# EugenHotaj/pytorch-generative

Measured on AMD Instinct MI355X. Metric: training images/sec (ImageGPT 8-block/4-head/16-embed, 28x28x1), higher is better.
Workload: dtype f32; 1 GPU; BASELINE.json configs[1]: ImageGPT 8 blocks / 4 heads / 16 embed on 28x28x1 binarised-MNIST-shaped synthetic; one step = zero_grad + fwd + BCE + bwd + global grad-norm + Adam + lr decay (reference trainer.py:173-193); per_gpu_batch=1024, global_batch=1024, parallelism=dp1, launch=hipGraph replay

## Files before the change

include/pg_hip.h:

```cpp
#ifndef PG_HIP_H_
#define PG_HIP_H_

#include <stddef.h>
#include <stdint.h>

#ifdef __cplusplus
extern "C" {
#endif

#define PG_ABI_VERSION 1

#define PG_EINVAL (-1)
#define PG_ESHAPE (-2)

#define PG_MAX_TAPS 64

#define PG_ACT_NONE 0
#define PG_ACT_RELU 1
#define PG_ACT_ELU 2
#define PG_ACT_GELU 3
#define PG_ACT_ELU_OUT 4

#define PG_GATE_TANH 0
#define PG_GATE_IDENTITY 1
// ... 70 lines not shown
                       long k_bs, long v_bs, long o_bs, long do_bs, long dq_bs, long dk_bs,
                       long dv_bs, int strict, void* stream);

int pg_causal_attn_bwd_dq(const float* q, const float* k, const float* v, const float* o,
                          const float* d_o, const float* lse2, float* delta, float* dq, float* dk,
                          float* dv, int N, int heads, int L, int dk_dim, int dv_dim, long q_bs,
                          long k_bs, long v_bs, long o_bs, long do_bs, long dq_bs, long dk_bs,
                          long dv_bs, int strict, void* stream);
int pg_causal_attn_bwd_dkv(const float* q, const float* k, const float* v, const float* o,
                           const float* d_o, const float* lse2, float* delta, float* dq, float* dk,
                           float* dv, int N, int heads, int L, int dk_dim, int dv_dim, long q_bs,
                           long k_bs, long v_bs, long o_bs, long do_bs, long dq_bs, long dk_bs,
                           long dv_bs, int strict, void* stream);

int pg_attn_fused_bwd(int enable);

#define PG_FEATURE_IDENTITY 0
#define PG_FEATURE_ELU1 1
size_t pg_linear_attn_workspace_floats(int N, int heads, int L, int dk, int dv, int backward);
int pg_linear_attn_fwd(const float* q, const float* k, const float* v, float* out, float* den, float* ws,
                       size_t ws_floats, int N, int heads, int L, int dk, int dv, long q_bs, long kv_bs,
                       long o_bs, int feature, void* stream);
int pg_linear_attn_bwd(const float* q, const float* k, const float* v, const float* out, const float* den,
                       const float* g, float* dq, float* dk, float* dv, float* ws, size_t ws_floats, int N,
                       int heads, int L, int dk_dim, int dv_dim, long q_bs, long kv_bs, long o_bs, int feature,
                       void* stream);

size_t pg_masked_linear_workspace_floats(int N, int in, int out, int dgrad);
int pg_masked_linear_fwd(const float* x, float* w, const float* b, const int* deg_in, const int* deg_out, int strict,
                         float* y, int N, int in, int out, int relu, float* ws, size_t ws_floats, void* stream);
// ... 145 lines not shown
```

pytorch-generative_amd/csrc/attention.hip:

```cpp
#include <stdlib.h>

#include "attention_args.h"

namespace {

constexpr float NEG_BIG = -1.0e30f;
constexpr float POS_BIG = 1.0e30f;
constexpr int QPL = 2;

using AttnArgs = PgAttnArgs;

__device__ __forceinline__ float fast_exp2(float x) { return __builtin_amdgcn_exp2f(x); }

template <int DK, int DV> struct Cfg {
  static constexpr int RS = DK + DV;
  static constexpr int RS2 = DK + DV + 4;
  static constexpr int CH = (RS <= 8) ? 8 : ((RS <= 16) ? 4 : 2);
  static constexpr int CH2 = (CH > 2) ? CH / 2 : 2;
};

template <int DA, int DB, int RS>
__device__ __forceinline__ void stage_rows(float* __restrict__ tile, const float* __restrict__ a,
                                           int da, const float* __restrict__ b, int db, int L,
                                           int m0, int KT, int tid, int nthreads) {
// ... 472 lines not shown
static bool use_mfma_attention() {
  static const bool on = []() {
    const char* e = PG_AB_ENV("PG_ATTN_MFMA");
    return !(e && e[0] == '0');
  }();
  return on;
}

static int launch_any(int which, AttnArgs& a, hipStream_t st) {
  static const int mask = []() { const char* e = PG_AB_ENV("PG_ATTN_MFMA_MASK"); return e ? atoi(e) : 7; }();
  const int bit = which == K_FWD ? 1 : (which == K_DQ ? 2 : 4);
  if (use_mfma_attention() && (mask & bit) && pg_attn_mfma_launch(which, a, st) == 1) return 0;
  return launch_attn(which, a, st);
}

PG_EXPORT int pg_causal_attn_fwd(const float* q, const float* k, const float* v, float* o,
                                 float* lse2, int N, int heads, int L, int dk, int dv, long q_bs,
                                 long k_bs, long v_bs, long o_bs, int strict, void* stream) {
  PG_REQUIRE(q && k && v && o && lse2, PG_EINVAL, "pg_causal_attn_fwd: null pointer");
  int rc = check_dims("pg_causal_attn_fwd", N, heads, L, dk, dv, strict);
  if (rc) return rc;
  AttnArgs a = {};
  a.q = q; a.k = k; a.v = v; a.o_out = o; a.lse2_out = lse2;
  a.N = N; a.heads = heads; a.L = L; a.dk_dim = dk; a.dv_dim = dv; a.strict = strict;
  a.q_bs = q_bs; a.k_bs = k_bs; a.v_bs = v_bs; a.o_bs = o_bs;
  a.scale = 1.f / sqrtf((float)dk);
  a.scale2 = a.scale * 1.44269504088896340736f;
  rc = launch_any(K_FWD, a, (hipStream_t)stream);
  PG_REQUIRE(rc == 0, rc, "pg_causal_attn_fwd: head dims (%d, %d) at L = %d are not instantiated: pad them to multiples of 16 and L to a multiple of 16 (ops.causal_attention does)", dk, dv, L);
  PG_LAUNCH_CHECK("pg_causal_attn_fwd");
  return 0;
}

namespace {
int attn_bwd_impl(int which_mask, const float* q, const float* k, const float* v, const float* o,
                  const float* d_o, const float* lse2, float* delta, float* dq, float* dk, float* dv,
                  int N, int heads, int L, int dk_dim, int dv_dim, long q_bs, long k_bs, long v_bs,
                  long o_bs, long do_bs, long dq_bs, long dk_bs, long dv_bs, int strict, void* stream) {
  PG_REQUIRE(q && k && v && o && d_o && lse2 && delta && dq && dk && dv, PG_EINVAL,
             "pg_causal_attn_bwd: null pointer");
  int rc = check_dims("pg_causal_attn_bwd", N, heads, L, dk_dim, dv_dim, strict);
  if (rc) return rc;
  AttnArgs a = {};
  a.q = q; a.k = k; a.v = v; a.o = o; a.d_o = d_o; a.lse2_in = lse2; a.delta = delta;
  a.dq = dq; a.dk = dk; a.dv = dv;
  a.N = N; a.heads = heads; a.L = L; a.dk_dim = dk_dim; a.dv_dim = dv_dim; a.strict = strict;
  a.q_bs = q_bs; a.k_bs = k_bs; a.v_bs = v_bs; a.o_bs = o_bs; a.do_bs = do_bs;
  a.dq_bs = dq_bs; a.dk_bs = dk_bs; a.dv_bs = dv_bs;
  a.scale = 1.f / sqrtf((float)dk_dim);
  a.scale2 = a.scale * 1.44269504088896340736f;
  if (which_mask == 3 && use_mfma_attention() && pg_attn_mfma_launch(PG_ATTN_BWD, a, (hipStream_t)stream) == 1) {
    PG_LAUNCH_CHECK("pg_causal_attn_bwd(fused)");
    return 0;
  }
  if (which_mask & 1) {
    rc = launch_any(K_DQ, a, (hipStream_t)stream);
    PG_REQUIRE(rc == 0, rc, "pg_causal_attn_bwd: head dims (%d, %d) at L = %d are not instantiated (see pg_causal_attn_fwd)", dk_dim, dv_dim, L);
    PG_LAUNCH_CHECK("pg_causal_attn_bwd(dq)");
  }
  if (which_mask & 2) {
    rc = launch_any(K_DKV, a, (hipStream_t)stream);
    PG_REQUIRE(rc == 0, rc, "pg_causal_attn_bwd: head dims (%d, %d) at L = %d are not instantiated (see pg_causal_attn_fwd)", dk_dim, dv_dim, L);
    PG_LAUNCH_CHECK("pg_causal_attn_bwd(dkv)");
  }
  return 0;
// ... 17 lines not shown
                                    float* dk, float* dv, int N, int heads, int L, int dk_dim,
                                    int dv_dim, long q_bs, long k_bs, long v_bs, long o_bs,
                                    long do_bs, long dq_bs, long dk_bs, long dv_bs, int strict,
                                    void* stream) {
  return attn_bwd_impl(1, PG_ATTN_BWD_ARGS);
}

PG_EXPORT int pg_causal_attn_bwd_dkv(const float* q, const float* k, const float* v, const float* o,
                                     const float* d_o, const float* lse2, float* delta, float* dq,
                                     float* dk, float* dv, int N, int heads, int L, int dk_dim,
                                     int dv_dim, long q_bs, long k_bs, long v_bs, long o_bs,
                                     long do_bs, long dq_bs, long dk_bs, long dv_bs, int strict,
                                     void* stream) {
  return attn_bwd_impl(2, PG_ATTN_BWD_ARGS);
}
```

pytorch-generative_amd/csrc/attention_args.h:

```cpp
#pragma once
#include "common.h"

struct PgAttnArgs {
  const float* q; const float* k; const float* v; const float* o; const float* d_o;
  const float* lse2_in;
  float* o_out; float* lse2_out; float* delta; float* dq; float* dk; float* dv;
  int N, heads, L, dk_dim, dv_dim, strict;
  long q_bs, k_bs, v_bs, o_bs, do_bs, dq_bs, dk_bs, dv_bs;
  float scale, scale2;
  int blocks_per_wg;
  int kt, kt2;
  int lp, vec;
  unsigned char bcount[8];
  unsigned char blist[8][16];
};

enum { PG_ATTN_FWD = 0, PG_ATTN_DQ = 1, PG_ATTN_DKV = 2, PG_ATTN_BWD = 3  };

int pg_attn_mfma_launch(int which, const PgAttnArgs& a, hipStream_t st);
```

pytorch-generative_amd/csrc/attention_mfma.hip:

```cpp
#include <stdio.h>
#include <stdlib.h>

#include <type_traits>

#include "attention_args.h"

namespace {

typedef float f32x4 __attribute__((ext_vector_type(4)));
constexpr float NEG_BIG = -1.0e30f;
constexpr float POS_BIG = 1.0e30f;
constexpr float PSUM_TH = 1024.0f;

typedef __bf16 bf16x8 __attribute__((ext_vector_type(8)));
#define MFMA16(A, B, C) __builtin_amdgcn_mfma_f32_16x16x4f32((A), (B), (C), 0, 0, 0)
#define MFMA16B(A, B, C) __builtin_amdgcn_mfma_f32_16x16x32_bf16((A), (B), (C), 0, 0, 0)
#define MFMA4(A, B, C) __builtin_amdgcn_mfma_f32_4x4x1f32((A), (B), (C), 0, 0, 0)

__device__ __forceinline__ float ex2(float x) { return __builtin_amdgcn_exp2f(x); }

__device__ __forceinline__ void quad_all(float x, float (&out)[4]) {
  const int v = __float_as_int(x);
  out[0] = __int_as_float(__builtin_amdgcn_update_dpp(0, v, 0x00, 0xf, 0xf, true));
  out[1] = __int_as_float(__builtin_amdgcn_update_dpp(0, v, 0x55, 0xf, 0xf, true));
// ... 96 lines not shown

struct Ids {
  int wave, lane, qi, g, jc, qb4;
};
__device__ __forceinline__ Ids ids() {
  Ids d;
  d.wave = __builtin_amdgcn_readfirstlane(threadIdx.x >> 6);
  d.lane = threadIdx.x & 63;
  d.qi = d.lane & 15;
  d.g = d.lane >> 4;
  d.jc = d.lane & 3;
  d.qb4 = ((d.lane >> 2) & 3) * 4;
  return d;
}

__global__ void __launch_bounds__(512) attn_fwd_m44_kernel(const PgAttnArgs a) {
  extern __shared__ float4 lds4[];
  const int Lp = a.lp;
  bf16x8* kc0 = reinterpret_cast<bf16x8*>(lds4);
  bf16x8* kc2 = kc0 + Lp;
  float* vt = reinterpret_cast<float*>(kc2 + Lp);
  bf16x8* ones = reinterpret_cast<bf16x8*>(vt + 4 * Lp);
  const Ids d = ids();
  const int qi = d.qi, g = d.g, jc = d.jc;
  const int h = blockIdx.y, n = blockIdx.z;
  const int L = a.L;
  const int NB = (L + 63) >> 6;

  const float* qp = a.q + (size_t)n * a.q_bs + (size_t)h * 4 * L;
  const float* kp = a.k + (size_t)n * a.k_bs + (size_t)h * 4 * L;
  const float* vp = a.v + (size_t)n * a.v_bs + (size_t)h * 4 * L;
  float* op = a.o_out + (size_t)n * a.o_bs + (size_t)h * 4 * L;
  float* lsep = a.lse2_out + ((size_t)n * a.heads + h) * L;

  const int rows = 64 * NB;
  const int nmine = a.bcount[d.wave];
  for (int m0 = 0; m0 < rows; m0 += 2 * blockDim.x) {
    float kx[2][4], vx[2][4];
#pragma unroll
    for (int u = 0; u < 2; ++u) {
      const int m = m0 + u * blockDim.x + threadIdx.x;
      load_row4(kx[u], kp, L, m);
      load_row4(vx[u], vp, L, m);
    }
#pragma unroll
    for (int u = 0; u < 2; ++u) {
      const int m = m0 + u * blockDim.x + threadIdx.x;
      if (m < rows) {
        put_chunks(kc0, kc2, m, kx[u]);
#pragma unroll
        for (int dd = 0; dd < 4; ++dd) vt[dd * Lp + m] = vx[u][dd];
      }
    }
  }
  if (threadIdx.x == 0) *ones = ones_chunk();
  __syncthreads();
  if (nmine == 0) return;
  const bf16x8* abase = g == 3 ? ones : (g == 2 ? kc2 : kc0) + qi;
  const int astride = g == 3 ? 0 : 1;

  const f32x4 zero4 = {0.f, 0.f, 0.f, 0.f};
#pragma unroll 1
  for (int it = 0; it < nmine; ++it) {
    const int blk = a.blist[d.wave][it];
    const int q0 = 64 * blk;
    const int ngrp = min(4, (L - q0 + 15) >> 4);

    float mcur[4], lsum[4];
    bf16x8 bq[4];
    f32x4 acc[4];
    int qidx[4];
#pragma unroll
    for (int t = 0; t < 4; ++t) {
      qidx[t] = q0 + 16 * t + qi;
      float qv[4];
      load_row4(qv, qp, L, qidx[t]);
#pragma unroll
      for (int dd = 0; dd < 4; ++dd) qv[dd] *= a.scale2;
      mcur[t] = 0.f;
// ... 79 lines not shown

#pragma unroll
    for (int t = 0; t < 4; ++t) {
      if (t < ngrp) {
        const float l = gsum(lsum[t]);
        float iq[4], ov[4];
        quad_all(l > 0.f ? 1.f / l : 0.f, iq);
#pragma unroll
        for (int i = 0; i < 4; ++i) ov[i] = gsum(acc[t][i]) * iq[i];
        if (g == 0) {
          store_rows4(op + (size_t)jc * L, L, q0 + 16 * t + d.qb4, a.vec, ov[0], ov[1], ov[2], ov[3]);
          if (qidx[t] < L) lsep[qidx[t]] = l > 0.f ? mcur[t] + log2f(l) : POS_BIG;
        }
      }
    }
  }
}

__global__ void __launch_bounds__(512) attn_dq_m44_kernel(const PgAttnArgs a) {
  extern __shared__ float4 lds4[];
  const int Lp = a.lp;
  bf16x8* kc0 = reinterpret_cast<bf16x8*>(lds4);
  bf16x8* kc2 = kc0 + Lp;
  bf16x8* vc0 = kc2 + Lp;
  bf16x8* vc2 = vc0 + Lp;
  float* kt = reinterpret_cast<float*>(vc2 + Lp);
  bf16x8* ones = reinterpret_cast<bf16x8*>(kt + 4 * Lp);
  const Ids d = ids();
  const int qi = d.qi, g = d.g, jc = d.jc;
  const int h = blockIdx.y, n = blockIdx.z;
  const int L = a.L;
  const int NB = (L + 63) >> 6;

  const float* qp = a.q + (size_t)n * a.q_bs + (size_t)h * 4 * L;
  const float* kp = a.k + (size_t)n * a.k_bs + (size_t)h * 4 * L;
  const float* vp = a.v + (size_t)n * a.v_bs + (size_t)h * 4 * L;
  const float* op = a.o + (size_t)n * a.o_bs + (size_t)h * 4 * L;
  const float* gp = a.d_o + (size_t)n * a.do_bs + (size_t)h * 4 * L;
  float* dqp = a.dq + (size_t)n * a.dq_bs + (size_t)h * 4 * L;
  const size_t row = ((size_t)n * a.heads + h) * L;

  const int rows = 64 * NB;
  const int nmine = a.bcount[d.wave];
  for (int m0 = 0; m0 < rows; m0 += 2 * blockDim.x) {
    float kx[2][4], vx[2][4];
#pragma unroll
    for (int u = 0; u < 2; ++u) {
      const int m = m0 + u * blockDim.x + threadIdx.x;
      load_row4(kx[u], kp, L, m);
      load_row4(vx[u], vp, L, m);
    }
#pragma unroll
    for (int u = 0; u < 2; ++u) {
      const int m = m0 + u * blockDim.x + threadIdx.x;
      if (m < rows) {
        put_chunks(kc0, kc2, m, kx[u]);
        put_chunks(vc0, vc2, m, vx[u]);
#pragma unroll
        for (int dd = 0; dd < 4; ++dd) kt[dd * Lp + m] = kx[u][dd];
      }
    }
  }
  if (threadIdx.x == 0) *ones = ones_chunk();
  __syncthreads();
  if (nmine == 0) return;
  const bf16x8* kbase = g == 3 ? ones : (g == 2 ? kc2 : kc0) + qi;
  const bf16x8* vbase = g == 3 ? ones : (g == 2 ? vc2 : vc0) + qi;
  const int astride = g == 3 ? 0 : 1;

  const f32x4 zero4 = {0.f, 0.f, 0.f, 0.f};
#pragma unroll 1
  for (int it = 0; it < nmine; ++it) {
    const int blk = a.blist[d.wave][it];
    const int q0 = 64 * blk;
    const int ngrp = min(4, (L - q0 + 15) >> 4);

    bf16x8 bq[4], bg[4];
    f32x4 acc[4];
    int qidx[4];
#pragma unroll
    for (int t = 0; t < 4; ++t) {
      qidx[t] = q0 + 16 * t + qi;
      const bool ok = qidx[t] < L;
      float qv[4], gv[4], ov[4], dl = 0.f;
      load_row4(qv, qp, L, qidx[t]);
      load_row4(gv, gp, L, qidx[t]);
      load_row4(ov, op, L, qidx[t]);
      const float lse = ok ? a.lse2_in[row + qidx[t]] : POS_BIG;
// ... 46 lines not shown
      step(k0, f, I<0>{}, B<false>{});
    }
    step(q0, fn, I<0>{}, B<true>{});
    if (ngrp > 1) step(q0 + 16, frag(q0 + 16), I<1>{}, B<true>{});
    if (ngrp > 2) step(q0 + 32, frag(q0 + 32), I<2>{}, B<true>{});
    if (ngrp > 3) step(q0 + 48, frag(q0 + 48), I<3>{}, B<true>{});
#pragma unroll
    for (int t = 0; t < 4; ++t) {
      if (t < ngrp) {
        float o4[4];
#pragma unroll
        for (int i = 0; i < 4; ++i) o4[i] = gsum(acc[t][i]) * a.scale;
        if (g == 0) store_rows4(dqp + (size_t)jc * L, L, q0 + 16 * t + d.qb4, a.vec, o4[0], o4[1], o4[2], o4[3]);
      }
    }
  }
}

template <bool BF16S>
__global__ void __launch_bounds__(512) attn_dkv_m44_kernel(const PgAttnArgs a) {
  extern __shared__ float4 lds4[];
  const int Lp = a.lp;
  bf16x8* qc0 = reinterpret_cast<bf16x8*>(lds4);
  bf16x8* qc2 = qc0 + Lp;
  float* qt = reinterpret_cast<float*>(lds4) + (BF16S ? 8 * Lp : 0);
  float* gt = qt + 4 * Lp;
  float* nlse = gt + 4 * Lp;
  float* ndel = nlse + Lp;
  const Ids d = ids();
  const int qi = d.qi, g = d.g, jc = d.jc;
  const int h = blockIdx.y, n = blockIdx.z;
  const int L = a.L;
  const int NB = (L + 63) >> 6;

  const float* qp = a.q + (size_t)n * a.q_bs + (size_t)h * 4 * L;
  const float* kp = a.k + (size_t)n * a.k_bs + (size_t)h * 4 * L;
  const float* vp = a.v + (size_t)n * a.v_bs + (size_t)h * 4 * L;
  const float* gp = a.d_o + (size_t)n * a.do_bs + (size_t)h * 4 * L;
  float* dkp = a.dk + (size_t)n * a.dk_bs + (size_t)h * 4 * L;
  float* dvp = a.dv + (size_t)n * a.dv_bs + (size_t)h * 4 * L;
  const size_t row = ((size_t)n * a.heads + h) * L;

  const int r0 = 0, r1 = 64 * NB;
  const int nmine = a.bcount[d.wave];
  for (int m0 = r0; m0 < r1; m0 += 2 * blockDim.x) {
    float qx[2][4], gx[2][4], lx[2], dx[2];
#pragma unroll
    for (int u = 0; u < 2; ++u) {
      const int m = m0 + u * blockDim.x + threadIdx.x;
      load_row4(qx[u], qp, L, m);
      load_row4(gx[u], gp, L, m);
      const int mc = m < L ? m : L - 1;
      lx[u] = a.lse2_in[row + mc];
      dx[u] = a.delta[row + mc];
    }
#pragma unroll
    for (int u = 0; u < 2; ++u) {
      const int m = m0 + u * blockDim.x + threadIdx.x;
      if (m < r1) {
#pragma unroll
        for (int dd = 0; dd < 4; ++dd) {
          qt[dd * Lp + m] = qx[u][dd];
          gt[dd * Lp + m] = gx[u][dd];
        }
        if (BF16S) put_chunks(qc0, qc2, m, qx[u]);
        nlse[m] = m < L ? -lx[u] : NEG_BIG;
        ndel[m] = m < L ? -dx[u] : 0.f;
      }
    }
  }
  __syncthreads();
  if (nmine == 0) return;
  const int q_end = ((L + 15) >> 4) << 4;
  const bf16x8* qbase = (g == 2 ? qc2 : qc0) + qi;

  const f32x4 zero4 = {0.f, 0.f, 0.f, 0.f};
#pragma unroll 1
  for (int it = 0; it < nmine; ++it) {
    const int blk = a.blist[d.wave][it];
    const int kb0 = 64 * blk;
    const int ngrp = min(4, (L - kb0 + 15) >> 4);

    float kf[4], vf[4];
    bf16x8 bk[4];
    f32x4 acck[4], accv[4];
    int kidx[4];
#pragma unroll
    for (int t = 0; t < 4; ++t) {
      kidx[t] = kb0 + 16 * t + qi;
      const bool ok = kidx[t] < L;
      const int kc = ok ? kidx[t] : L - 1;
      kf[t] = ok ? kp[(size_t)g * L + kc] * a.scale2 : 0.f;
      vf[t] = ok ? vp[(size_t)g * L + kc] : 0.f;
      if (BF16S) {
// ... 64 lines not shown
#pragma unroll
    for (int t = 0; t < 4; ++t) {
      if (t < ngrp) {
        float k4[4], v4[4];
#pragma unroll
        for (int i = 0; i < 4; ++i) {
          k4[i] = gsum(acck[t][i]) * a.scale;
          v4[i] = gsum(accv[t][i]);
        }
        if (g == 0) {
          store_rows4(dkp + (size_t)jc * L, L, kb0 + 16 * t + d.qb4, a.vec, k4[0], k4[1], k4[2], k4[3]);
          store_rows4(dvp + (size_t)jc * L, L, kb0 + 16 * t + d.qb4, a.vec, v4[0], v4[1], v4[2], v4[3]);
        }
      }
    }
  }
}

__device__ __forceinline__ bf16x8 resident_operand_k(const float (&x)[4], int kg) {
  bf16x8 v;
#pragma unroll
  for (int dd = 0; dd < 4; ++dd) {
    const Split3 s = split3(x[dd]);
    v[dd] = kg == 1 ? s.m : (kg == 3 ? s.l : s.h);
    v[4 + dd] = kg == 0 ? s.h : (kg == 1 ? s.m : (__bf16)0.f);
  }
  if (kg == 2) { v[4] = v[5] = v[6] = (__bf16)1.f; }
  return v;
}

__device__ __forceinline__ void put_row32(bf16x8* __restrict__ w1, bf16x8* __restrict__ w2, int row,
// ... 28 lines not shown
  const int h = blockIdx.y, n = blockIdx.z;
  const int L = a.L;
  const int NB = (L + 63) >> 6;

  const float* qp = a.q + (size_t)n * a.q_bs + (size_t)h * 4 * L;
  const float* kp = a.k + (size_t)n * a.k_bs + (size_t)h * 4 * L;
  const float* vp = a.v + (size_t)n * a.v_bs + (size_t)h * 4 * L;
  const float* op = a.o + (size_t)n * a.o_bs + (size_t)h * 4 * L;
  const float* gp = a.d_o + (size_t)n * a.do_bs + (size_t)h * 4 * L;
  float* dqp = a.dq + (size_t)n * a.dq_bs + (size_t)h * 4 * L;
  float* dkp = a.dk + (size_t)n * a.dk_bs + (size_t)h * 4 * L;
  float* dvp = a.dv + (size_t)n * a.dv_bs + (size_t)h * 4 * L;
  const size_t row = ((size_t)n * a.heads + h) * L;

  const int r1 = 64 * NB;
  const int nmine = a.bcount[d.wave];
  for (int m0 = 0; m0 < r1; m0 += 2 * blockDim.x) {
    float qx[2][4], gx[2][4], ox[2][4], lx[2];
#pragma unroll
    for (int u = 0; u < 2; ++u) {
      const int m = m0 + u * blockDim.x + threadIdx.x;
      load_row4(qx[u], qp, L, m);
      load_row4(gx[u], gp, L, m);
      load_row4(ox[u], op, L, m);
      lx[u] = a.lse2_in[row + (m < L ? m : L - 1)];
    }
#pragma unroll
    for (int u = 0; u < 2; ++u) {
      const int m = m0 + u * blockDim.x + threadIdx.x;
      if (m < r1) {
        float dl = 0.f;
#pragma unroll
        for (int dd = 0; dd < 4; ++dd) {
          qt[dd * Lp + m] = qx[u][dd];
          gt[dd * Lp + m] = gx[u][dd];
          dqa[dd * Lp + m] = 0.f;
          dl = fmaf(gx[u][dd], ox[u][dd], dl);
        }
        put_row32(qw1, qw2, m, qx[u], m < L ? -lx[u] : NEG_BIG);
        ndel[m] = -dl;
      }
    }
  }
  __syncthreads();
  const int q_end = ((L + 15) >> 4) << 4;
  const bf16x8* qbase = (g == 2 ? qw2 : qw1) + qi;
  float* scr_w = scr + 4 * (16 * g + ((qi + 2 * g) & 15));
  const float* scr_r[4];
#pragma unroll
  for (int sl = 0; sl < 4; ++sl)
    scr_r[sl] = scr + 4 * (16 * (qi >> 2) + ((g + 4 * sl + 2 * (qi >> 2)) & 15)) + (qi & 3);
  float* red_w = scr + 64 * g + 16 * jc + d.qb4;
  const float* red_r = scr + d.lane;
  unsigned int* dq_slot = reinterpret_cast<unsigned int*>(dqa + (d.lane >> 4) * Lp + (d.lane & 15));

  const f32x4 zero4 = {0.f, 0.f, 0.f, 0.f};
#pragma unroll 1
  for (int it = 0; it < nmine; ++it) {
    const int blk = a.blist[d.wave][it];
    const int kb0 = 64 * blk;
    const int ngrp = min(4, (L - kb0 + 15) >> 4);

    float vf[4];
    bf16x8 bk[4];
    f32x4 kq[4];
    f32x4 acck[4], accv[4];
    int kidx[4];
    int g_row = g, jc_row = jc;
    asm volatile("" : "+v"(g_row), "+v"(jc_row));
#pragma unroll
    for (int t = 0; t < 4; ++t) {
      kidx[t] = kb0 + 16 * t + qi;
      const bool ok = kidx[t] < L;
      vf[t] = ok ? vp[(size_t)g_row * L + kidx[t]] : 0.f;
// ... 96 lines not shown
      if (t < ngrp) {
        float k4[4], v4[4];
#pragma unroll
        for (int i = 0; i < 4; ++i) {
          k4[i] = gsum(acck[t][i]) * a.scale;
          v4[i] = gsum(accv[t][i]);
        }
        if (g == 0) {
          int jcs = jc;
          asm volatile("" : "+v"(jcs));
          store_rows4(dkp + (size_t)jcs * L, L, kb0 + 16 * t + d.qb4, a.vec, k4[0], k4[1], k4[2], k4[3]);
          store_rows4(dvp + (size_t)jcs * L, L, kb0 + 16 * t + d.qb4, a.vec, v4[0], v4[1], v4[2], v4[3]);
        }
      }
    }
  }
  __syncthreads();
#pragma unroll
  for (int dd = 0; dd < 4; ++dd)
    for (int m = threadIdx.x; m < L; m += blockDim.x) dqp[(size_t)dd * L + m] = dqa[dd * Lp + m] * a.scale;
}

bool aligned16(const void* p) { return (reinterpret_cast<uintptr_t>(p) & 15) == 0; }

}

struct AttnWaveCfg { int w[3]; };
static void attn_waves(int* w) {
  static const AttnWaveCfg cfg = []() {
    AttnWaveCfg c = {{4, 8, 4}};
    if (const char* e = PG_AB_ENV("PG_ATTN_WAVES")) {
      int f = 0, q = 0, k = 0;
      if (sscanf(e, "%d,%d,%d", &f, &q, &k) == 3 && f >= 1 && f <= 8 && q >= 1 && q <= 8 && k >= 1 && k <= 8)
        c = {{f, q, k}};
    }
// ... 3 lines not shown
}

int pg_attn_k4_launch(int which, const PgAttnArgs& a, hipStream_t st);

#include <atomic>
static std::atomic<int>& fused_bwd_flag() {
  static std::atomic<int> flag([]() { const char* e = PG_AB_ENV("PG_ATTN_FUSED_BWD"); return (e && e[0] == '0') ? 0 : 1; }());
  return flag;
}
static bool pg_attn_fused_bwd_enabled() { return fused_bwd_flag().load(std::memory_order_relaxed) != 0; }
PG_EXPORT int pg_attn_fused_bwd(int enable) {
  if (enable < 0) return fused_bwd_flag().load(std::memory_order_relaxed);
  return fused_bwd_flag().exchange(enable ? 1 : 0, std::memory_order_relaxed);
}

int pg_attn_mfma_launch(int which, const PgAttnArgs& a0, hipStream_t st) {
  if (which == PG_ATTN_BWD) {
    if (!pg_attn_fused_bwd_enabled()) return 0;
    if (a0.dk_dim != 4 || a0.dv_dim != 4) {
      static const bool k4_fused = []() { const char* e = PG_AB_ENV("PG_ATTN_FUSED_BWD_K4"); return !(e && e[0] == '0'); }();
      return k4_fused ? pg_attn_k4_launch(which, a0, st) : 0;
    }
  }
  if (a0.dk_dim != 4 || a0.dv_dim != 4) return pg_attn_k4_launch(which, a0, st);
  PgAttnArgs a = a0;
  const int NB = (a.L + 63) / 64;
  a.lp = 64 * NB + 16;
  static const bool dkv_bf16 = []() { const char* e = PG_AB_ENV("PG_ATTN_DKV_BF16"); return !(e && e[0] == '0'); }();
  const size_t planes = which == PG_ATTN_BWD ? 21
                        : which == PG_ATTN_DKV ? (dkv_bf16 ? 18 : 10) : (which == PG_ATTN_DQ ? 20 : 12);
  int wcfg[3];
  attn_waves(wcfg);
  static const int bwd_waves = []() {
    const char* e = PG_AB_ENV("PG_ATTN_BWD_WAVES");
    const int v = e ? atoi(e) : 8;
    return v >= 1 && v <= 8 ? v : 8;
  }();
  int W = which == PG_ATTN_BWD ? bwd_waves : wcfg[which];
  const size_t shmem = planes * (size_t)a.lp * sizeof(float) + (which == PG_ATTN_BWD ? 8 * 1024 : 16);
  if (shmem > 160 * 1024) return 0;
  if (which == PG_ATTN_DKV && dkv_bf16 && !PG_AB_ENV("PG_ATTN_WAVES")) W = 8;
  if (which == PG_ATTN_FWD && (long)a.N * a.heads <= 512 && !PG_AB_ENV("PG_ATTN_WAVES")) W = 8;
  if (W > NB) W = NB;
  if ((NB + W - 1) / W > 16) return 0;
  long load[8] = {0, 0, 0, 0, 0, 0, 0, 0};
  for (int w = 0; w < 8; ++w) a.bcount[w] = 0;
  for (int rank = NB - 1; rank >= 0; --rank) {
    const int blk = (which == PG_ATTN_DKV || which == PG_ATTN_BWD) ? NB - 1 - rank : rank;
    int best = 0;
    for (int w = 1; w < W; ++w)
      if (load[w] < load[best] && a.bcount[w] < 16) best = w;
    if (a.bcount[best] >= 16) return 0;
    a.blist[best][a.bcount[best]++] = (unsigned char)blk;
    load[best] += 4 * rank + 5;
  }
  a.vec = a.L % 4 == 0 ? 1 : 0;
  if (which == PG_ATTN_FWD)
    a.vec = a.vec && aligned16(a.o_out) && a.o_bs % 4 == 0;
  else if (which == PG_ATTN_DQ)
    a.vec = a.vec && aligned16(a.dq) && a.dq_bs % 4 == 0;
  else
    a.vec = a.vec && aligned16(a.dk) && aligned16(a.dv) && a.dk_bs % 4 == 0 && a.dv_bs % 4 == 0;
  dim3 grid(1u, (unsigned)a.heads, (unsigned)a.N);
  dim3 block((unsigned)(64 * W));
  const void* fn = which == PG_ATTN_FWD  ? reinterpret_cast<const void*>(attn_fwd_m44_kernel)
                   : which == PG_ATTN_BWD ? (a.lp == 848 ? reinterpret_cast<const void*>(attn_bwd_m44_kernel<848>)
                                             : a.lp == 1040 ? reinterpret_cast<const void*>(attn_bwd_m44_kernel<1040>)
                                                            : reinterpret_cast<const void*>(attn_bwd_m44_kernel<0>))
                   : which == PG_ATTN_DQ ? reinterpret_cast<const void*>(attn_dq_m44_kernel)
                   : dkv_bf16            ? reinterpret_cast<const void*>(attn_dkv_m44_kernel<true>)
// ... 19 lines not shown
```

pytorch-generative_amd/pytorch_generative_amd/_lib.py:

```python

import ctypes
import os

_HERE = os.path.dirname(os.path.abspath(__file__))
LIB_PATH = os.environ.get("PG_HIP_LIB") or os.path.join(_HERE, "lib", "libpg_hip.so")

ABI_VERSION = 1

c_f = ctypes.c_void_p
c_i = ctypes.c_int
c_l = ctypes.c_long
c_z = ctypes.c_size_t
c_s = ctypes.c_void_p
c_ip = ctypes.POINTER(ctypes.c_int)
c_flt = ctypes.c_float

SIGNATURES = {
    "pg_abi_version": (c_i, []),
    "pg_last_error": (ctypes.c_char_p, []),
    "pg_conv2d_taps": (
        c_i,
        [c_f, c_f, c_f, c_f, c_f, c_i, c_i, c_i, c_i, c_i, c_i, c_i, c_i, c_ip, c_ip, c_i, c_f, c_i,
         c_s],
    ),
# ... 102 lines not shown
    "pg_avgpool2_bwd": (c_i, [c_f, c_f, c_i, c_i, c_i, c_s]),
    "pg_upsample2_fwd": (c_i, [c_f, c_f, c_i, c_i, c_i, c_s]),
    "pg_upsample2_bwd": (c_i, [c_f, c_f, c_i, c_i, c_i, c_s]),
    "pg_phase_split2": (c_i, [c_f, c_f, c_i, c_i, c_i, c_i, c_s]),
    "pg_gauss_head_fwd": (c_i, [c_f, c_f, c_f, c_f, c_f, c_i, c_i, c_i, c_l, c_l, c_i, c_s]),
    "pg_gauss_head_bwd": (c_i, [c_f, c_f, c_f, c_f, c_f, c_f, c_f, c_i, c_i, c_i, c_l, c_l, c_i, c_s]),
    "pg_vec_mean_accum": (c_i, [c_f, c_i, c_f, c_s]),
    "pg_fill_scaled": (c_i, [c_f, c_flt, c_f, c_i, c_s]),
    "pg_sumsq_accum": (c_i, [c_f, c_z, c_f, c_s]),
    "pg_adam_prepare": (c_i, [c_f, c_s]),
    "pg_sumsq_partial_count": (c_i, [c_z]),
    "pg_sumsq_partials": (c_i, [c_f, c_z, c_f, c_s]),
    "pg_adam_prepare_ordered": (c_i, [c_f, c_f, c_i, c_s]),
    "pg_adam_step": (c_i, [c_f, c_f, c_f, c_f, c_z, c_f, c_flt, c_flt, c_flt, c_s]),
    "pg_attn_fused_bwd": (c_i, [c_i]),
    "pg_concat_elu_fwd": (c_i, [c_f, c_f, c_i, c_l, c_s]),
    "pg_concat_elu_bwd": (c_i, [c_f, c_f, c_f, c_i, c_l, c_s]),
    "pg_dmol_fwd": (c_i, [c_f, c_f, c_f, c_i, c_i, c_i, c_s]),
    "pg_dmol_bwd": (c_i, [c_f, c_f, c_f, c_f, c_i, c_i, c_i, c_s]),
    "pg_copy_rows": (c_i, [c_f, c_f, c_l, c_l, c_l, c_l, c_i, c_s]),
    "pg_comm_unique_id": (c_i, [ctypes.c_char_p]),
    "pg_comm_init": (c_i, [c_i, c_i, ctypes.c_char_p]),
    "pg_comm_world": (c_i, []),
    "pg_comm_rccl_version": (c_i, []),
    "pg_allreduce_sum": (c_i, [c_f, c_z, c_i, c_s]),
    "pg_broadcast": (c_i, [c_f, c_z, c_i, c_i, c_s]),
    "pg_comm_destroy": (c_i, []),
}
COMM_ID_BYTES = 128
DTYPE_F32 = 0
# ... 70 lines not shown
```

Baseline: 100,000 images/s.

## Refine MFMA attention block-to-wave plan with SIMD-aware search and caching

Moves the MFMA causal-attention block-to-wave assignment into a plan builder that is cached per (which, L, few-units). After the greedy LPT pass, the builder runs a bounded DFS that also balances load across the 4 SIMDs (waves w and w+4 share a SIMD), aiming to shorten the critical path of the most loaded SIMD. It also adds rotation-based wave-to-list mapping and timestamp instrumentation, both of which are only active via new exported entry points or the debug build. The search costs host time only on cache misses, and the rotation logic adds a readfirstlane plus a branch in each kernel.

```diff
diff --git a/include/pg_hip.h b/include/pg_hip.h
--- a/include/pg_hip.h
+++ b/include/pg_hip.h
@@ -108,6 +108,17 @@
                            long dv_bs, int strict, void* stream);
 
 int pg_attn_fused_bwd(int enable);
+
+int pg_attn_mfma_plan(int which, int L, long n_units, int* lists_out, int* counts_out, long* loads_out);
+int pg_attn_mfma_list_of(int wave, int workgroup, int rot, int W);
+int pg_causal_attn_fwd_rot(const float* q, const float* k, const float* v, float* o, float* lse2,
+                           int N, int heads, int L, int dk, int dv, long q_bs, long k_bs, long v_bs,
+                           long o_bs, int strict, int rot, void* stream);
+int pg_causal_attn_bwd_rot(int which, const float* q, const float* k, const float* v, const float* o,
+                           const float* d_o, const float* lse2, float* delta, float* dq, float* dk,
+                           float* dv, int N, int heads, int L, int dk_dim, int dv_dim, long q_bs,
+                           long k_bs, long v_bs, long o_bs, long do_bs, long dq_bs, long dk_bs,
+                           long dv_bs, int strict, int rot, void* stream);
 
 #define PG_FEATURE_IDENTITY 0
 #define PG_FEATURE_ELU1 1
diff --git a/pytorch-generative_amd/csrc/attention.hip b/pytorch-generative_amd/csrc/attention.hip
--- a/pytorch-generative_amd/csrc/attention.hip
+++ b/pytorch-generative_amd/csrc/attention.hip
@@ -510,9 +510,9 @@
   return launch_attn(which, a, st);
 }
 
-PG_EXPORT int pg_causal_attn_fwd(const float* q, const float* k, const float* v, float* o,
-                                 float* lse2, int N, int heads, int L, int dk, int dv, long q_bs,
-                                 long k_bs, long v_bs, long o_bs, int strict, void* stream) {
+namespace {
+int attn_fwd_impl(const float* q, const float* k, const float* v, float* o, float* lse2, int N, int heads, int L,
+                  int dk, int dv, long q_bs, long k_bs, long v_bs, long o_bs, int strict, int rot, void* stream) {
   PG_REQUIRE(q && k && v && o && lse2, PG_EINVAL, "pg_causal_attn_fwd: null pointer");
   int rc = check_dims("pg_causal_attn_fwd", N, heads, L, dk, dv, strict);
   if (rc) return rc;
@@ -522,17 +522,31 @@
   a.q_bs = q_bs; a.k_bs = k_bs; a.v_bs = v_bs; a.o_bs = o_bs;
   a.scale = 1.f / sqrtf((float)dk);
   a.scale2 = a.scale * 1.44269504088896340736f;
+  a.rot_fixed = rot < 0 ? 0 : rot + 1;
   rc = launch_any(K_FWD, a, (hipStream_t)stream);
   PG_REQUIRE(rc == 0, rc, "pg_causal_attn_fwd: head dims (%d, %d) at L = %d are not instantiated: pad them to multiples of 16 and L to a multiple of 16 (ops.causal_attention does)", dk, dv, L);
   PG_LAUNCH_CHECK("pg_causal_attn_fwd");
   return 0;
 }
+}
+
+PG_EXPORT int pg_causal_attn_fwd(const float* q, const float* k, const float* v, float* o,
+                                 float* lse2, int N, int heads, int L, int dk, int dv, long q_bs,
+                                 long k_bs, long v_bs, long o_bs, int strict, void* stream) {
+  return attn_fwd_impl(q, k, v, o, lse2, N, heads, L, dk, dv, q_bs, k_bs, v_bs, o_bs, strict, -1, stream);
+}
+
+PG_EXPORT int pg_causal_attn_fwd_rot(const float* q, const float* k, const float* v, float* o,
+                                     float* lse2, int N, int heads, int L, int dk, int dv, long q_bs,
+                                     long k_bs, long v_bs, long o_bs, int strict, int rot, void* stream) {
+  return attn_fwd_impl(q, k, v, o, lse2, N, heads, L, dk, dv, q_bs, k_bs, v_bs, o_bs, strict, rot, stream);
+}
 
 namespace {
 int attn_bwd_impl(int which_mask, const float* q, const float* k, const float* v, const float* o,
                   const float* d_o, const float* lse2, float* delta, float* dq, float* dk, float* dv,
                   int N, int heads, int L, int dk_dim, int dv_dim, long q_bs, long k_bs, long v_bs,
-                  long o_bs, long do_bs, long dq_bs, long dk_bs, long dv_bs, int strict, void* stream) {
+                  long o_bs, long do_bs, long dq_bs, long dk_bs, long dv_bs, int strict, void* stream, int rot = -1) {
   PG_REQUIRE(q && k && v && o && d_o && lse2 && delta && dq && dk && dv, PG_EINVAL,
              "pg_causal_attn_bwd: null pointer");
   int rc = check_dims("pg_causal_attn_bwd", N, heads, L, dk_dim, dv_dim, strict);
@@ -545,6 +559,7 @@
   a.dq_bs = dq_bs; a.dk_bs = dk_bs; a.dv_bs = dv_bs;
   a.scale = 1.f / sqrtf((float)dk_dim);
   a.scale2 = a.scale * 1.44269504088896340736f;
+  a.rot_fixed = rot < 0 ? 0 : rot + 1;
   if (which_mask == 3 && use_mfma_attention() && pg_attn_mfma_launch(PG_ATTN_BWD, a, (hipStream_t)stream) == 1) {
     PG_LAUNCH_CHECK("pg_causal_attn_bwd(fused)");
     return 0;
@@ -592,3 +607,13 @@
                                      void* stream) {
   return attn_bwd_impl(2, PG_ATTN_BWD_ARGS);
 }
+
+PG_EXPORT int pg_causal_attn_bwd_rot(int which, const float* q, const float* k, const float* v, const float* o,
+                                     const float* d_o, const float* lse2, float* delta, float* dq,
+                                     float* dk, float* dv, int N, int heads, int L, int dk_dim,
+                                     int dv_dim, long q_bs, long k_bs, long v_bs, long o_bs,
+                                     long do_bs, long dq_bs, long dk_bs, long dv_bs, int strict, int rot,
+                                     void* stream) {
+  PG_REQUIRE(which >= 1 && which <= 3, PG_EINVAL, "pg_causal_attn_bwd_rot: which must be 1, 2 or 3");
+  return attn_bwd_impl(which, PG_ATTN_BWD_ARGS, rot);
+}
diff --git a/pytorch-generative_amd/csrc/attention_args.h b/pytorch-generative_amd/csrc/attention_args.h
--- a/pytorch-generative_amd/csrc/attention_args.h
+++ b/pytorch-generative_amd/csrc/attention_args.h
@@ -13,8 +13,30 @@
   int lp, vec;
   unsigned char bcount[8];
   unsigned char blist[8][16];
+  int rot_fixed;
+#ifdef PG_AB
+  unsigned long long* dbg;
+  unsigned int dbg_waves;
+#endif
 };
+
+__host__ __device__ inline unsigned pg_attn_rot_of(unsigned id, unsigned W) { return (id + (id >> 3) + (id >> 8)) % W; }
+__host__ __device__ inline unsigned pg_attn_list_of(unsigned wave, unsigned rot, unsigned W) {
+  if (W == 8) return wave < 4 ? ((wave + rot) & 3) : 4 + ((wave + rot + (rot >> 2)) & 3);
+  const unsigned x = wave + rot;
+  return x >= W ? x - W : x;
+}
+#define PG_ATTN_DBG_WORDS 24
 
 enum { PG_ATTN_FWD = 0, PG_ATTN_DQ = 1, PG_ATTN_DKV = 2, PG_ATTN_BWD = 3  };
 
 int pg_attn_mfma_launch(int which, const PgAttnArgs& a, hipStream_t st);
+
+struct PgAttnPlan {
+  int W;
+  unsigned char bcount[8];
+  unsigned char blist[8][16];
+  long load[8];
+  size_t shmem;
+};
+PgAttnPlan pg_attn_mfma_make_plan(int which, int L, long n_units);
diff --git a/pytorch-generative_amd/csrc/attention_mfma.hip b/pytorch-generative_amd/csrc/attention_mfma.hip
--- a/pytorch-generative_amd/csrc/attention_mfma.hip
+++ b/pytorch-generative_amd/csrc/attention_mfma.hip
@@ -134,6 +134,44 @@
   return d;
 }
 
+__device__ __forceinline__ int my_list(const PgAttnArgs& a, int wave) {
+  if (a.rot_fixed == 0) return wave;
+  const unsigned W = blockDim.x >> 6;
+  unsigned rot = a.rot_fixed > 0 ? (unsigned)(a.rot_fixed - 1) % W : 0u;
+#ifdef PG_AB
+  if (a.rot_fixed < 0) rot = pg_attn_rot_of(blockIdx.y + gridDim.y * blockIdx.z, W);
+#endif
+  return __builtin_amdgcn_readfirstlane((int)pg_attn_list_of((unsigned)wave, rot, W));
+}
+
+#ifdef PG_AB
+__device__ __forceinline__ unsigned long long* stamp_begin(const PgAttnArgs& a, int wave, int li, int nmine) {
+  const unsigned long long t = __builtin_amdgcn_s_memtime();
+  if (!a.dbg) return nullptr;
+  const unsigned wg = blockIdx.y + gridDim.y * blockIdx.z;
+  const unsigned long long w = (unsigned long long)wg * 8 + (unsigned)wave;
+  if (w >= a.dbg_waves) return nullptr;
+  unsigned long long* r = a.dbg + w * PG_ATTN_DBG_WORDS;
+  if ((threadIdx.x & 63) == 0) {
+    r[0] = (unsigned long long)wg | ((unsigned long long)wave << 32) | ((unsigned long long)li << 40) |
+           ((unsigned long long)(blockDim.x >> 6) << 48);
+    r[1] = (unsigned long long)__builtin_amdgcn_s_getreg(4 | (31 << 11)) |
+           ((unsigned long long)__builtin_amdgcn_s_getreg(20 | (31 << 11)) << 32);
+    r[2] = t;
+    r[5] = (unsigned long long)nmine;
+  }
+  return r;
+}
+__device__ __forceinline__ void stamp(unsigned long long* r, int slot) {
+  if (r && (threadIdx.x & 63) == 0 && slot < PG_ATTN_DBG_WORDS) r[slot] = __builtin_amdgcn_s_memtime();
+}
+#define PG_STAMP_BEGIN(a, wave, li, nmine) unsigned long long* const stamps_ = stamp_begin(a, wave, li, nmine)
+#define PG_STAMP(slot) stamp(stamps_, slot)
+#else
+#define PG_STAMP_BEGIN(a, wave, li, nmine) ((void)0)
+#define PG_STAMP(slot) ((void)0)
+#endif
+
 __global__ void __launch_bounds__(512) attn_fwd_m44_kernel(const PgAttnArgs a) {
   extern __shared__ float4 lds4[];
   const int Lp = a.lp;
@@ -154,7 +192,9 @@
   float* lsep = a.lse2_out + ((size_t)n * a.heads + h) * L;
 
   const int rows = 64 * NB;
-  const int nmine = a.bcount[d.wave];
+  const int li = my_list(a, d.wave);
+  const int nmine = a.bcount[li];
+  PG_STAMP_BEGIN(a, d.wave, li, nmine);
   for (int m0 = 0; m0 < rows; m0 += 2 * blockDim.x) {
     float kx[2][4], vx[2][4];
 #pragma unroll
@@ -175,14 +215,18 @@
   }
   if (threadIdx.x == 0) *ones = ones_chunk();
   __syncthreads();
-  if (nmine == 0) return;
+  PG_STAMP(3);
+  if (nmine == 0) {
+    PG_STAMP(4);
+    return;
+  }
   const bf16x8* abase = g == 3 ? ones : (g == 2 ? kc2 : kc0) + qi;
   const int astride = g == 3 ? 0 : 1;
 
   const f32x4 zero4 = {0.f, 0.f, 0.f, 0.f};
 #pragma unroll 1
   for (int it = 0; it < nmine; ++it) {
-    const int blk = a.blist[d.wave][it];
+    const int blk = a.blist[li][it];
     const int q0 = 64 * blk;
     const int ngrp = min(4, (L - q0 + 15) >> 4);
 
@@ -292,7 +336,9 @@
         }
       }
     }
-  }
+    PG_STAMP(6 + it);
+  }
+  PG_STAMP(4);
 }
 
 __global__ void __launch_bounds__(512) attn_dq_m44_kernel(const PgAttnArgs a) {
@@ -319,7 +365,9 @@
   const size_t row = ((size_t)n * a.heads + h) * L;
 
   const int rows = 64 * NB;
-  const int nmine = a.bcount[d.wave];
+  const int li = my_list(a, d.wave);
+  const int nmine = a.bcount[li];
+  PG_STAMP_BEGIN(a, d.wave, li, nmine);
   for (int m0 = 0; m0 < rows; m0 += 2 * blockDim.x) {
     float kx[2][4], vx[2][4];
 #pragma unroll
@@ -341,7 +389,11 @@
   }
   if (threadIdx.x == 0) *ones = ones_chunk();
   __syncthreads();
-  if (nmine == 0) return;
+  PG_STAMP(3);
+  if (nmine == 0) {
+    PG_STAMP(4);
+    return;
+  }
   const bf16x8* kbase = g == 3 ? ones : (g == 2 ? kc2 : kc0) + qi;
   const bf16x8* vbase = g == 3 ? ones : (g == 2 ? vc2 : vc0) + qi;
   const int astride = g == 3 ? 0 : 1;
@@ -349,7 +401,7 @@
   const f32x4 zero4 = {0.f, 0.f, 0.f, 0.f};
 #pragma unroll 1
   for (int it = 0; it < nmine; ++it) {
-    const int blk = a.blist[d.wave][it];
+    const int blk = a.blist[li][it];
     const int q0 = 64 * blk;
     const int ngrp = min(4, (L - q0 + 15) >> 4);
 
@@ -426,7 +478,9 @@
         if (g == 0) store_rows4(dqp + (size_t)jc * L, L, q0 + 16 * t + d.qb4, a.vec, o4[0], o4[1], o4[2], o4[3]);
       }
     }
-  }
+    PG_STAMP(6 + it);
+  }
+  PG_STAMP(4);
 }
 
 template <bool BF16S>
@@ -454,7 +508,9 @@
   const size_t row = ((size_t)n * a.heads + h) * L;
 
   const int r0 = 0, r1 = 64 * NB;
-  const int nmine = a.bcount[d.wave];
+  const int li = my_list(a, d.wave);
+  const int nmine = a.bcount[li];
+  PG_STAMP_BEGIN(a, d.wave, li, nmine);
   for (int m0 = r0; m0 < r1; m0 += 2 * blockDim.x) {
     float qx[2][4], gx[2][4], lx[2], dx[2];
 #pragma unroll
@@ -482,14 +538,18 @@
     }
   }
   __syncthreads();
-  if (nmine == 0) return;
+  PG_STAMP(3);
+  if (nmine == 0) {
+    PG_STAMP(4);
+    return;
+  }
   const int q_end = ((L + 15) >> 4) << 4;
   const bf16x8* qbase = (g == 2 ? qc2 : qc0) + qi;
 
   const f32x4 zero4 = {0.f, 0.f, 0.f, 0.f};
 #pragma unroll 1
   for (int it = 0; it < nmine; ++it) {
-    const int blk = a.blist[d.wave][it];
+    const int blk = a.blist[li][it];
     const int kb0 = 64 * blk;
     const int ngrp = min(4, (L - kb0 + 15) >> 4);
 
@@ -584,7 +644,9 @@
         }
       }
     }
-  }
+    PG_STAMP(6 + it);
+  }
+  PG_STAMP(4);
 }
 
 __device__ __forceinline__ bf16x8 resident_operand_k(const float (&x)[4], int kg) {
@@ -643,7 +705,9 @@
   const size_t row = ((size_t)n * a.heads + h) * L;
 
   const int r1 = 64 * NB;
-  const int nmine = a.bcount[d.wave];
+  const int li = my_list(a, d.wave);
+  const int nmine = a.bcount[li];
+  PG_STAMP_BEGIN(a, d.wave, li, nmine);
   for (int m0 = 0; m0 < r1; m0 += 2 * blockDim.x) {
     float qx[2][4], gx[2][4], ox[2][4], lx[2];
 #pragma unroll
@@ -672,6 +736,7 @@
     }
   }
   __syncthreads();
+  PG_STAMP(3);
   const int q_end = ((L + 15) >> 4) << 4;
   const bf16x8* qbase = (g == 2 ? qw2 : qw1) + qi;
   float* scr_w = scr + 4 * (16 * g + ((qi + 2 * g) & 15));
@@ -686,7 +751,7 @@
   const f32x4 zero4 = {0.f, 0.f, 0.f, 0.f};
 #pragma unroll 1
   for (int it = 0; it < nmine; ++it) {
-    const int blk = a.blist[d.wave][it];
+    const int blk = a.blist[li][it];
     const int kb0 = 64 * blk;
     const int ngrp = min(4, (L - kb0 + 15) >> 4);
 
@@ -813,11 +878,14 @@
         }
       }
     }
-  }
+    PG_STAMP(6 + it);
+  }
+  PG_STAMP(22);
   __syncthreads();
 #pragma unroll
   for (int dd = 0; dd < 4; ++dd)
     for (int m = threadIdx.x; m < L; m += blockDim.x) dqp[(size_t)dd * L + m] = dqa[dd * Lp + m] * a.scale;
+  PG_STAMP(4);
 }
 
 bool aligned16(const void* p) { return (reinterpret_cast<uintptr_t>(p) & 15) == 0; }
@@ -851,19 +919,28 @@
   return fused_bwd_flag().exchange(enable ? 1 : 0, std::memory_order_relaxed);
 }
 
-int pg_attn_mfma_launch(int which, const PgAttnArgs& a0, hipStream_t st) {
-  if (which == PG_ATTN_BWD) {
-    if (!pg_attn_fused_bwd_enabled()) return 0;
-    if (a0.dk_dim != 4 || a0.dv_dim != 4) {
-      static const bool k4_fused = []() { const char* e = PG_AB_ENV("PG_ATTN_FUSED_BWD_K4"); return !(e && e[0] == '0'); }();
-      return k4_fused ? pg_attn_k4_launch(which, a0, st) : 0;
-    }
-  }
-  if (a0.dk_dim != 4 || a0.dv_dim != 4) return pg_attn_k4_launch(which, a0, st);
-  PgAttnArgs a = a0;
-  const int NB = (a.L + 63) / 64;
-  a.lp = 64 * NB + 16;
-  static const bool dkv_bf16 = []() { const char* e = PG_AB_ENV("PG_ATTN_DKV_BF16"); return !(e && e[0] == '0'); }();
+static bool dkv_bf16_enabled() {
+  static const bool on = []() { const char* e = PG_AB_ENV("PG_ATTN_DKV_BF16"); return !(e && e[0] == '0'); }();
+  return on;
+}
+
+constexpr long PG_ATTN_COST_STEP = 4, PG_ATTN_COST_BASE = 5;
+
+static PgAttnPlan make_plan(int which, int L, long n_units);
+PgAttnPlan pg_attn_mfma_make_plan(int which, int L, long n_units) {
+  if (which < PG_ATTN_FWD || which > PG_ATTN_BWD || L <= 0 || n_units <= 0) return PgAttnPlan{};
+  struct Slot { int L; bool few; PgAttnPlan p; };
+  static thread_local Slot slots[4] = {};
+  Slot& sl = slots[which];
+  const bool few = n_units <= 512;
+  if (sl.L != L || sl.few != few) sl = Slot{L, few, make_plan(which, L, n_units)};
+  return sl.p;
+}
+static PgAttnPlan make_plan(int which, int L, long n_units) {
+  PgAttnPlan p = {};
+  const int NB = (L + 63) / 64;
+  const size_t lp = 64 * (size_t)NB + 16;
+  const bool dkv_bf16 = dkv_bf16_enabled();
   const size_t planes = which == PG_ATTN_BWD ? 21
                         : which == PG_ATTN_DKV ? (dkv_bf16 ? 18 : 10) : (which == PG_ATTN_DQ ? 20 : 12);
   int wcfg[3];
@@ -874,23 +951,132 @@
     return v >= 1 && v <= 8 ? v : 8;
   }();
   int W = which == PG_ATTN_BWD ? bwd_waves : wcfg[which];
-  const size_t shmem = planes * (size_t)a.lp * sizeof(float) + (which == PG_ATTN_BWD ? 8 * 1024 : 16);
-  if (shmem > 160 * 1024) return 0;
+  p.shmem = planes * lp * sizeof(float) + (which == PG_ATTN_BWD ? 8 * 1024 : 16);
+  if (p.shmem > 160 * 1024) return p;
   if (which == PG_ATTN_DKV && dkv_bf16 && !PG_AB_ENV("PG_ATTN_WAVES")) W = 8;
-  if (which == PG_ATTN_FWD && (long)a.N * a.heads <= 512 && !PG_AB_ENV("PG_ATTN_WAVES")) W = 8;
+  if (which == PG_ATTN_FWD && n_units <= 512 && !PG_AB_ENV("PG_ATTN_WAVES")) W = 8;
   if (W > NB) W = NB;
-  if ((NB + W - 1) / W > 16) return 0;
+  if ((NB + W - 1) / W > 16) return p;
+  const bool rev = which == PG_ATTN_DKV || which == PG_ATTN_BWD;
+  int rk[8][16];
+  int cnt[8] = {0, 0, 0, 0, 0, 0, 0, 0};
   long load[8] = {0, 0, 0, 0, 0, 0, 0, 0};
-  for (int w = 0; w < 8; ++w) a.bcount[w] = 0;
+  auto cost = [](int rank) { return PG_ATTN_COST_STEP * rank + PG_ATTN_COST_BASE; };
   for (int rank = NB - 1; rank >= 0; --rank) {
-    const int blk = (which == PG_ATTN_DKV || which == PG_ATTN_BWD) ? NB - 1 - rank : rank;
     int best = 0;
     for (int w = 1; w < W; ++w)
-      if (load[w] < load[best] && a.bcount[w] < 16) best = w;
-    if (a.bcount[best] >= 16) return 0;
-    a.blist[best][a.bcount[best]++] = (unsigned char)blk;
-    load[best] += 4 * rank + 5;
-  }
+      if (load[w] < load[best] && cnt[w] < 16) best = w;
+    if (cnt[best] >= 16) return p;
+    rk[best][cnt[best]++] = rank;
+    load[best] += cost(rank);
+  }
+  static const bool refine = []() { const char* e = PG_AB_ENV("PG_ATTN_REFINE"); return !(e && e[0] == '0'); }();
+  if (refine && W > 1) {
+    const int S = W < 4 ? W : 4;
+    long total = 0, list_cap = 0, simd_lpt = 0;
+    int count_cap = 0;
+    for (int w = 0; w < W; ++w) {
+      total += load[w];
+      list_cap = load[w] > list_cap ? load[w] : list_cap;
+      count_cap = cnt[w] > count_cap ? cnt[w] : count_cap;
+    }
+    for (int sd = 0; sd < S; ++sd) {
+      const long v = load[sd] + (sd + 4 < W ? load[sd + 4] : 0);
+      simd_lpt = v > simd_lpt ? v : simd_lpt;
+    }
+    long cur[8], scur[4];
+    int ccnt[8], where[128];
+    int budget = 30000;
+    long bound = 0;
+    auto dfs = [&](auto&& self, int i) -> bool {
+      if (i == NB) return true;
+      if (--budget < 0) return false;
+      const long c = cost(NB - 1 - i);
+      for (int w = 0; w < W; ++w) {
+        if (cur[w] + c > list_cap || ccnt[w] >= count_cap || scur[w & 3] + c > bound) continue;
+        bool dup = false;
+        for (int u = 0; u < w && !dup; ++u)
+          dup = cur[u] == cur[w] && ccnt[u] == ccnt[w] && scur[u & 3] == scur[w & 3];
+        if (dup) continue;
+        cur[w] += c; scur[w & 3] += c; ++ccnt[w]; where[i] = w;
+        if (self(self, i + 1)) return true;
+        cur[w] -= c; scur[w & 3] -= c; --ccnt[w];
+      }
+      return false;
+    };
+    for (bound = (total + S - 1) / S; bound < simd_lpt && budget > 0; ++bound) {
+      for (int w = 0; w < 8; ++w) cur[w] = 0, ccnt[w] = 0;
+      for (int sd = 0; sd < 4; ++sd) scur[sd] = 0;
+      if (!dfs(dfs, 0)) continue;
+      for (int w = 0; w < 8; ++w) cnt[w] = 0, load[w] = 0;
+      for (int i = 0; i < NB; ++i) {
+        rk[where[i]][cnt[where[i]]++] = NB - 1 - i;
+        load[where[i]] += cost(NB - 1 - i);
+      }
+      break;
+    }
+  }
+  for (int w = 0; w < W; ++w) {
+    p.bcount[w] = (unsigned char)cnt[w];
+    p.load[w] = load[w];
+    for (int x = 0; x < cnt[w]; ++x) p.blist[w][x] = (unsigned char)(rev ? NB - 1 - rk[w][x] : rk[w][x]);
+  }
+  p.W = W;
+  return p;
+}
+
+PG_EXPORT int pg_attn_mfma_plan(int which, int L, long n_units, int* lists_out, int* counts_out, long* loads_out) {
+  const PgAttnPlan p = pg_attn_mfma_make_plan(which, L, n_units);
+  for (int w = 0; w < 8; ++w) {
+    if (counts_out) counts_out[w] = w < p.W ? p.bcount[w] : 0;
+    if (loads_out) loads_out[w] = w < p.W ? p.load[w] : 0;
+    if (lists_out)
+      for (int x = 0; x < 16; ++x) lists_out[16 * w + x] = (w < p.W && x < p.bcount[w]) ? p.blist[w][x] : -1;
+  }
+  return p.W;
+}
+PG_EXPORT int pg_attn_mfma_list_of(int wave, int workgroup, int rot, int W) {
+  if (W < 1 || W > 8 || wave < 0 || wave >= W || workgroup < 0) return -1;
+  const unsigned r = rot >= 0 ? (unsigned)rot % (unsigned)W : 0u;
+  return (int)pg_attn_list_of((unsigned)wave, r, (unsigned)W);
+}
+
+#ifdef PG_AB
+static unsigned long long* g_attn_dbg = nullptr;
+static unsigned int g_attn_dbg_waves = 0;
+PG_EXPORT void pg_attn_dbg_buffer(void* dev_ptr, size_t bytes) {
+  g_attn_dbg = static_cast<unsigned long long*>(dev_ptr);
+  g_attn_dbg_waves = dev_ptr ? (unsigned int)(bytes / (PG_ATTN_DBG_WORDS * sizeof(unsigned long long))) : 0;
+}
+#endif
+
+int pg_attn_mfma_launch(int which, const PgAttnArgs& a0, hipStream_t st) {
+  if (which == PG_ATTN_BWD) {
+    if (!pg_attn_fused_bwd_enabled()) return 0;
+    if (a0.dk_dim != 4 || a0.dv_dim != 4) {
+      static const bool k4_fused = []() { const char* e = PG_AB_ENV("PG_ATTN_FUSED_BWD_K4"); return !(e && e[0] == '0'); }();
+      return k4_fused ? pg_attn_k4_launch(which, a0, st) : 0;
+    }
+  }
+  if (a0.dk_dim != 4 || a0.dv_dim != 4) return pg_attn_k4_launch(which, a0, st);
+  PgAttnArgs a = a0;
+  const PgAttnPlan plan = pg_attn_mfma_make_plan(which, a.L, (long)a.N * a.heads);
+  if (plan.W == 0) return 0;
+  const int W = plan.W;
+  const int NB = (a.L + 63) / 64;
+  a.lp = 64 * NB + 16;
+  const size_t shmem = plan.shmem;
+  const bool dkv_bf16 = dkv_bf16_enabled();
+  for (int w = 0; w < 8; ++w) {
+    a.bcount[w] = plan.bcount[w];
+    for (int x = 0; x < 16; ++x) a.blist[w][x] = plan.blist[w][x];
+  }
+#ifdef PG_AB
+  a.dbg = g_attn_dbg;
+  a.dbg_waves = g_attn_dbg_waves;
+  if (const char* e = PG_AB_ENV("PG_ATTN_ROT"))
+    if (!a.rot_fixed) a.rot_fixed = e[0] == 'i' ? -1 : atoi(e) + 1;
+#endif
   a.vec = a.L % 4 == 0 ? 1 : 0;
   if (which == PG_ATTN_FWD)
     a.vec = a.vec && aligned16(a.o_out) && a.o_bs % 4 == 0;
diff --git a/pytorch-generative_amd/pytorch_generative_amd/_lib.py b/pytorch-generative_amd/pytorch_generative_amd/_lib.py
--- a/pytorch-generative_amd/pytorch_generative_amd/_lib.py
+++ b/pytorch-generative_amd/pytorch_generative_amd/_lib.py
@@ -140,6 +140,17 @@
     "pg_adam_prepare_ordered": (c_i, [c_f, c_f, c_i, c_s]),
     "pg_adam_step": (c_i, [c_f, c_f, c_f, c_f, c_z, c_f, c_flt, c_flt, c_flt, c_s]),
     "pg_attn_fused_bwd": (c_i, [c_i]),
+    "pg_attn_mfma_plan": (c_i, [c_i, c_i, c_l, c_ip, c_ip, ctypes.POINTER(ctypes.c_long)]),
+    "pg_attn_mfma_list_of": (c_i, [c_i, c_i, c_i, c_i]),
+    "pg_causal_attn_fwd_rot": (
+        c_i,
+        [c_f, c_f, c_f, c_f, c_f, c_i, c_i, c_i, c_i, c_i, c_l, c_l, c_l, c_l, c_i, c_i, c_s],
+    ),
+    "pg_causal_attn_bwd_rot": (
+        c_i,
+        [c_i, c_f, c_f, c_f, c_f, c_f, c_f, c_f, c_f, c_f, c_f, c_i, c_i, c_i, c_i, c_i, c_l, c_l, c_l,
+         c_l, c_l, c_l, c_l, c_l, c_i, c_i, c_s],
+    ),
     "pg_concat_elu_fwd": (c_i, [c_f, c_f, c_i, c_l, c_s]),
     "pg_concat_elu_bwd": (c_i, [c_f, c_f, c_f, c_i, c_l, c_s]),
     "pg_dmol_fwd": (c_i, [c_f, c_f, c_f, c_i, c_i, c_i, c_s]),
```

After: 100,200 images/s, median of 6. Within noise of the previous version (+0.2%).
